# carrenD/Medical-Cross-Modality-Domain-Adaptation

Measured on NVIDIA H100. Metric: slices_per_sec_full_adversarial_step_256x256x3, higher is better.
Workload: dtype f32 (wgmma bf16 hi/lo split x3, fp32 accumulate)

## Files before the change

medical-cross-modality-domain-adaptation_b200/csrc/conv_tc.cu:

```cuda
#include <cuda.h>
#include <cstdio>
#include <cstdlib>
#include <cuda_bf16.h>
#include "common.cuh"
#include "../../include/pnp_b200.h"

namespace {

constexpr int BLOCK_M = 128;
constexpr int BLOCK_K = 64;
constexpr int WGMMA_K = 16;
constexpr int CONSUMER_THREADS = 256;
constexpr int CONSUMER_WARPS = CONSUMER_THREADS / 32;
constexpr int TC_THREADS = CONSUMER_THREADS + 32;

__device__ __forceinline__ uint32_t smem_u32(const void* p) { return (uint32_t)__cvta_generic_to_shared(p); }

__device__ __forceinline__ void mbar_init(uint32_t bar, uint32_t count) {
  asm volatile("mbarrier.init.shared::cta.b64 [%0], %1;" ::"r"(bar), "r"(count));
}
__device__ __forceinline__ void mbar_expect_tx(uint32_t bar, uint32_t bytes) {
  asm volatile("mbarrier.arrive.expect_tx.shared::cta.b64 _, [%0], %1;" ::"r"(bar), "r"(bytes) : "memory");
}
__device__ __forceinline__ void mbar_arrive(uint32_t bar) {
  asm volatile("mbarrier.arrive.shared::cta.b64 _, [%0];" ::"r"(bar) : "memory");
}
__device__ __forceinline__ bool mbar_try_wait(uint32_t bar, uint32_t parity) {
  uint32_t ok;
  asm volatile(
      "{\n\t.reg .pred p;\n\t"
      "mbarrier.try_wait.parity.shared::cta.b64 p, [%1], %2;\n\t"
      "selp.u32 %0, 1, 0, p;\n\t}"
      : "=r"(ok)
      : "r"(bar), "r"(parity)
      : "memory");
  return ok != 0;
}
__device__ __forceinline__ unsigned long long globaltimer_ns() {
  unsigned long long t;
  asm volatile("mov.u64 %0, %globaltimer;" : "=l"(t));
  return t;
}
__device__ __forceinline__ void mbar_wait(uint32_t bar, uint32_t parity) {
  if (mbar_try_wait(bar, parity)) return;
  unsigned long long t0 = globaltimer_ns();
  while (!mbar_try_wait(bar, parity)) {
    if (globaltimer_ns() - t0 > 4000000000ull) __trap();
  }
}
__device__ __forceinline__ void fence_barrier_init() { asm volatile("fence.mbarrier_init.release.cluster;" ::: "memory"); }
__device__ __forceinline__ void consumer_sync() { asm volatile("bar.sync 1, %0;" ::"n"(CONSUMER_THREADS) : "memory"); }

__device__ __forceinline__ void tma_load_4d(uint32_t dst, const CUtensorMap* map, uint32_t bar, int c0, int c1, int c2, int c3) {
  asm volatile(
      "cp.async.bulk.tensor.4d.shared::cluster.global.tile.mbarrier::complete_tx::bytes [%0], [%1, {%3, %4, %5, %6}], [%2];"
      ::"r"(dst), "l"(map), "r"(bar), "r"(c0), "r"(c1), "r"(c2), "r"(c3)
      : "memory");
}
__device__ __forceinline__ void tma_load_2d(uint32_t dst, const CUtensorMap* map, uint32_t bar, int c0, int c1) {
  asm volatile(
      "cp.async.bulk.tensor.2d.shared::cluster.global.tile.mbarrier::complete_tx::bytes [%0], [%1, {%3, %4}], [%2];"
      ::"r"(dst), "l"(map), "r"(bar), "r"(c0), "r"(c1)
      : "memory");
}
__device__ __forceinline__ void tma_prefetch_desc(const CUtensorMap* map) {
  asm volatile("prefetch.tensormap [%0];" ::"l"(map) : "memory");
}

__device__ __forceinline__ void wgmma_fence() { asm volatile("wgmma.fence.sync.aligned;" ::: "memory"); }
__device__ __forceinline__ void wgmma_commit() { asm volatile("wgmma.commit_group.sync.aligned;" ::: "memory"); }
template <int N>
__device__ __forceinline__ void wgmma_wait() { asm volatile("wgmma.wait_group.sync.aligned %0;" ::"n"(N) : "memory"); }
template <int R>
__device__ __forceinline__ void fence_acc(float (&d)[R]) {
#pragma unroll
  for (int i = 0; i < R; ++i) asm volatile("" : "+f"(d[i])::"memory");
}


template <int TA, int TB>
__device__ __forceinline__ void wgmma_m64n16k16(float (&d)[8], uint64_t da, uint64_t db, int scale_d) {
  asm volatile(
      "{\n\t.reg .pred p;\n\tsetp.ne.b32 p, %10, 0;\n\t"
      "wgmma.mma_async.sync.aligned.m64n16k16.f32.bf16.bf16 {"
      "%0, %1, %2, %3, %4, %5, %6, %7"
      "}, %8, %9, p, 1, 1, %11, %12;\n\t}"
      : "+f"(d[0]), "+f"(d[1]), "+f"(d[2]), "+f"(d[3]), "+f"(d[4]), "+f"(d[5]), "+f"(d[6]), "+f"(d[7])
      : "l"(da), "l"(db), "r"(scale_d), "n"(TA), "n"(TB)
      : "memory");
}
template <int TA, int TB>
__device__ __forceinline__ void wgmma_m64n32k16(float (&d)[16], uint64_t da, uint64_t db, int scale_d) {
  asm volatile(
      "{\n\t.reg .pred p;\n\tsetp.ne.b32 p, %18, 0;\n\t"
      "wgmma.mma_async.sync.aligned.m64n32k16.f32.bf16.bf16 {"
      "%0, %1, %2, %3, %4, %5, %6, %7, %8, %9, %10, %11, %12, %13, %14, %15"
      "}, %16, %17, p, 1, 1, %19, %20;\n\t}"
      : "+f"(d[0]), "+f"(d[1]), "+f"(d[2]), "+f"(d[3]), "+f"(d[4]), "+f"(d[5]), "+f"(d[6]), "+f"(d[7]),
        "+f"(d[8]), "+f"(d[9]), "+f"(d[10]), "+f"(d[11]), "+f"(d[12]), "+f"(d[13]), "+f"(d[14]), "+f"(d[15])
      : "l"(da), "l"(db), "r"(scale_d), "n"(TA), "n"(TB)
      : "memory");
}
template <int TA, int TB>
__device__ __forceinline__ void wgmma_m64n64k16(float (&d)[32], uint64_t da, uint64_t db, int scale_d) {
  asm volatile(
      "{\n\t.reg .pred p;\n\tsetp.ne.b32 p, %34, 0;\n\t"
      "wgmma.mma_async.sync.aligned.m64n64k16.f32.bf16.bf16 {"
      "%0, %1, %2, %3, %4, %5, %6, %7, %8, %9, %10, %11, %12, %13, %14, %15, "
      "%16, %17, %18, %19, %20, %21, %22, %23, %24, %25, %26, %27, %28, %29, %30, %31"
      "}, %32, %33, p, 1, 1, %35, %36;\n\t}"
      : "+f"(d[0]), "+f"(d[1]), "+f"(d[2]), "+f"(d[3]), "+f"(d[4]), "+f"(d[5]), "+f"(d[6]), "+f"(d[7]),
        "+f"(d[8]), "+f"(d[9]), "+f"(d[10]), "+f"(d[11]), "+f"(d[12]), "+f"(d[13]), "+f"(d[14]), "+f"(d[15]),
        "+f"(d[16]), "+f"(d[17]), "+f"(d[18]), "+f"(d[19]), "+f"(d[20]), "+f"(d[21]), "+f"(d[22]), "+f"(d[23]),
        "+f"(d[24]), "+f"(d[25]), "+f"(d[26]), "+f"(d[27]), "+f"(d[28]), "+f"(d[29]), "+f"(d[30]), "+f"(d[31])
      : "l"(da), "l"(db), "r"(scale_d), "n"(TA), "n"(TB)
      : "memory");
}
template <int TA, int TB>
__device__ __forceinline__ void wgmma_m64n128k16(float (&d)[64], uint64_t da, uint64_t db, int scale_d) {
  asm volatile(
      "{\n\t.reg .pred p;\n\tsetp.ne.b32 p, %66, 0;\n\t"
      "wgmma.mma_async.sync.aligned.m64n128k16.f32.bf16.bf16 {"
      "%0, %1, %2, %3, %4, %5, %6, %7, %8, %9, %10, %11, %12, %13, %14, %15, "
      "%16, %17, %18, %19, %20, %21, %22, %23, %24, %25, %26, %27, %28, %29, %30, %31, "
      "%32, %33, %34, %35, %36, %37, %38, %39, %40, %41, %42, %43, %44, %45, %46, %47, "
      "%48, %49, %50, %51, %52, %53, %54, %55, %56, %57, %58, %59, %60, %61, %62, %63"
      "}, %64, %65, p, 1, 1, %67, %68;\n\t}"
      : "+f"(d[0]), "+f"(d[1]), "+f"(d[2]), "+f"(d[3]), "+f"(d[4]), "+f"(d[5]), "+f"(d[6]), "+f"(d[7]),
        "+f"(d[8]), "+f"(d[9]), "+f"(d[10]), "+f"(d[11]), "+f"(d[12]), "+f"(d[13]), "+f"(d[14]), "+f"(d[15]),
        "+f"(d[16]), "+f"(d[17]), "+f"(d[18]), "+f"(d[19]), "+f"(d[20]), "+f"(d[21]), "+f"(d[22]), "+f"(d[23]),
        "+f"(d[24]), "+f"(d[25]), "+f"(d[26]), "+f"(d[27]), "+f"(d[28]), "+f"(d[29]), "+f"(d[30]), "+f"(d[31]),
        "+f"(d[32]), "+f"(d[33]), "+f"(d[34]), "+f"(d[35]), "+f"(d[36]), "+f"(d[37]), "+f"(d[38]), "+f"(d[39]),
        "+f"(d[40]), "+f"(d[41]), "+f"(d[42]), "+f"(d[43]), "+f"(d[44]), "+f"(d[45]), "+f"(d[46]), "+f"(d[47]),
        "+f"(d[48]), "+f"(d[49]), "+f"(d[50]), "+f"(d[51]), "+f"(d[52]), "+f"(d[53]), "+f"(d[54]), "+f"(d[55]),
// ... 40 lines not shown
  int kchunks;
  int ntaps;
  short tap_oy[MAX_TAPS], tap_ox[MAX_TAPS];
  int tap_wrow[MAX_TAPS];
  int tw, th, tn;
  int tiles_x, tiles_y, tiles_n;
  int accumulate;
  PnpDropout drop;
  double* bn_sum;
  double* bn_sumsq;
  const float* ep_scale;
  const float* ep_shift;
  const float* ep_skip;
  int ep_skip_c, ep_skip_off, ep_act;
  uint16_t* out_hi;
  uint16_t* out_lo;
  int total_tiles;
  int rot_mul;
  int taps_inner;
  int ksplit;
  int nphases;
  struct Phase {
    short tap_begin, tap_count, py, px;
    int U, V, tiles_x, tiles_y, tile_base;
  } ph[16];
};

struct TileCoord {
  int x0, y0, img0, n0, tap_begin, tap_count, U, V, py, px, kb_begin, kb_count, mt;
};

template <int BLOCK_N>
__device__ __forceinline__ TileCoord decode_tile(const TcArgs& a, int t, int n_tiles) {
  TileCoord c;
  int tiles_x = a.tiles_x, tiles_y = a.tiles_y;
  int ks = 0;
  if (a.ksplit > 1) { ks = t % a.ksplit; t /= a.ksplit; }
  c.tap_begin = 0; c.tap_count = a.ntaps; c.U = a.U; c.V = a.V; c.py = a.out_py; c.px = a.out_px;
  if (a.nphases > 0) {
    int p = 0;
    while (p + 1 < a.nphases && t >= a.ph[p + 1].tile_base) ++p;
    t -= a.ph[p].tile_base;
    tiles_x = a.ph[p].tiles_x; tiles_y = a.ph[p].tiles_y;
    c.tap_begin = a.ph[p].tap_begin; c.tap_count = a.ph[p].tap_count;
    c.U = a.ph[p].U; c.V = a.ph[p].V; c.py = a.ph[p].py; c.px = a.ph[p].px;
  }
  int mt = t / n_tiles;
  c.mt = mt;
  c.n0 = (t - mt * n_tiles) * BLOCK_N;
  const int txi = mt % tiles_x;
  mt /= tiles_x;
  const int tyi = mt % tiles_y;
  const int tni = mt / tiles_y;
  c.x0 = txi * a.tw; c.y0 = tyi * a.th; c.img0 = tni * a.tn;
  const int nkb = c.tap_count * a.kchunks;
  if (a.ksplit > 1) {
    c.kb_begin = (int)((long long)nkb * ks / a.ksplit);
    c.kb_count = (int)((long long)nkb * (ks + 1) / a.ksplit) - c.kb_begin;
  } else {
    c.kb_begin = 0; c.kb_count = nkb;
  }
  return c;
}

__device__ __forceinline__ void kblock_of(const TcArgs& a, const TileCoord& tc, int i, int kchunks, int& tap, int& kc) {
  const int rot = (tc.kb_count >= 16) ? (int)(((long long)tc.mt * a.rot_mul) % tc.kb_count) : 0;
  int kr = i + rot;
  if (kr >= tc.kb_count) kr -= tc.kb_count;
  const int kb = tc.kb_begin + kr;
  int tl;
  if (a.taps_inner) { kc = kb / tc.tap_count; tl = kb - kc * tc.tap_count; }
  else { tl = kb / kchunks; kc = kb - tl * kchunks; }
  tap = tc.tap_begin + tl;
}

template <int BLOCK_N, int NTERMS, int BK>
struct TcCfg {
  static constexpr int A_TILE_BYTES = BLOCK_M * BK * 2;
  static constexpr int B_TILE_BYTES = BLOCK_N * BK * 2;
  static constexpr int NPLANES = (NTERMS == 1) ? 1 : 2;
  static constexpr int STAGE_BYTES = NPLANES * (A_TILE_BYTES + B_TILE_BYTES);
  static constexpr int STAGES_RAW = (200 * 1024) / STAGE_BYTES;
  static constexpr int STAGES = STAGES_RAW > 8 ? 8 : STAGES_RAW;
  static constexpr int STAT_BYTES = 2 * BLOCK_N * 8;
  static constexpr int SMEM_BYTES = STAGES * STAGE_BYTES + STAT_BYTES + 1024  + 256 ;
  static_assert(STAGES >= 2, "pipeline needs two stages");
  static_assert(SMEM_BYTES <= 227 * 1024, "H100 allows 227 KB of shared memory per block");
};

__device__ __forceinline__ uint32_t word_of(const uint4& r, int k) { return k == 0 ? r.x : k == 1 ? r.y : k == 2 ? r.z : r.w; }

template <int BLOCK_N, int NTERMS, int BK>
__global__ void __launch_bounds__(TC_THREADS, 1)
conv_tc_kernel(const __grid_constant__ CUtensorMap map_a_hi, const __grid_constant__ CUtensorMap map_a_lo,
               const __grid_constant__ CUtensorMap map_b_hi, const __grid_constant__ CUtensorMap map_b_lo,
               float* __restrict__ out, TcArgs a) {
  pnp_pdl_trigger();
  using Cfg = TcCfg<BLOCK_N, NTERMS, BK>;
  constexpr int A_TILE_BYTES = Cfg::A_TILE_BYTES;
  constexpr int STAGES = Cfg::STAGES;
  constexpr int ACC = BLOCK_N / 2;
  extern __shared__ uint8_t smem_raw[];
  uint8_t* smem = reinterpret_cast<uint8_t*>((reinterpret_cast<uintptr_t>(smem_raw) + 1023) & ~(uintptr_t)1023);
  double* stat = reinterpret_cast<double*>(smem + STAGES * Cfg::STAGE_BYTES);
  uint64_t* bars = reinterpret_cast<uint64_t*>(stat + 2 * BLOCK_N);

  const int warp = threadIdx.x >> 5;
  const int lane = threadIdx.x & 31;
  const int n_tiles = a.Cout / BLOCK_N;
  const int kchunks = a.kchunks;
  const bool bn_on = a.bn_sum != nullptr;

  if (threadIdx.x == 0) {
    tma_prefetch_desc(&map_a_hi);
    tma_prefetch_desc(&map_b_hi);
    if (NTERMS > 1) { tma_prefetch_desc(&map_a_lo); tma_prefetch_desc(&map_b_lo); }
    for (int s = 0; s < STAGES; ++s) {
      mbar_init(smem_u32(&bars[s]), 1);
      mbar_init(smem_u32(&bars[STAGES + s]), CONSUMER_WARPS);
    }
    fence_barrier_init();
  }
  for (int i = threadIdx.x; i < 2 * BLOCK_N; i += TC_THREADS) stat[i] = 0.0;
  __syncthreads();
  pnp_pdl_wait();

  if (warp == CONSUMER_WARPS) {
    if (lane == 0) {
      const uint32_t box_a_bytes = (uint32_t)(a.tw * a.th * a.tn) * BK * 2;
      const uint32_t tx_bytes = Cfg::NPLANES * (box_a_bytes + (uint32_t)Cfg::B_TILE_BYTES);
      int stage = 0;
      uint32_t phase = 0;
      for (int t = blockIdx.x; t < a.total_tiles; t += gridDim.x) {
        const TileCoord tc = decode_tile<BLOCK_N>(a, t, n_tiles);
        for (int i = 0; i < tc.kb_count; ++i) {
          int tap, kc;
          kblock_of(a, tc, i, kchunks, tap, kc);
          mbar_wait(smem_u32(&bars[STAGES + stage]), phase ^ 1);
          const uint32_t full = smem_u32(&bars[stage]);
          mbar_expect_tx(full, tx_bytes);
          uint8_t* st = smem + stage * Cfg::STAGE_BYTES;
          const int cx = tc.x0 * a.in_mul + a.tap_ox[tap];
          const int cy = tc.y0 * a.in_mul + a.tap_oy[tap];
          const int wrow = a.tap_wrow[tap] + tc.n0;
          tma_load_4d(smem_u32(st), &map_a_hi, full, kc * BK, cx, cy, tc.img0);
          tma_load_2d(smem_u32(st + Cfg::NPLANES * A_TILE_BYTES), &map_b_hi, full, kc * BK, wrow);
          if (NTERMS > 1) {
            tma_load_4d(smem_u32(st + A_TILE_BYTES), &map_a_lo, full, kc * BK, cx, cy, tc.img0);
            tma_load_2d(smem_u32(st + 2 * A_TILE_BYTES + Cfg::B_TILE_BYTES), &map_b_lo, full, kc * BK, wrow);
          }
          if (++stage == STAGES) { stage = 0; phase ^= 1; }
        }
      }
    }
    return;
  }

  const int wg = warp >> 2;
  const int q = lane & 3;
  const int cq = q * 2;
  const int per_img = a.th * a.tw;
  const bool drop_on = a.drop.seed_ptr != nullptr;
  unsigned long long seed = 0ull;
  if (drop_on) seed = *a.drop.seed_ptr;
  int stat_n0 = -1;
  auto flush_stats = [&]() {
    consumer_sync();
    for (int i = threadIdx.x; i < BLOCK_N; i += CONSUMER_THREADS) {
      atomicAdd(a.bn_sum + stat_n0 + i, stat[i]);
      atomicAdd(a.bn_sumsq + stat_n0 + i, stat[BLOCK_N + i]);
      stat[i] = 0.0;
      stat[BLOCK_N + i] = 0.0;
    }
    consumer_sync();
  };

  float acc[ACC];
  int stage = 0;
  uint32_t phase = 0;
  for (int t = blockIdx.x; t < a.total_tiles; t += gridDim.x) {
    const TileCoord tc = decode_tile<BLOCK_N>(a, t, n_tiles);
    const int n0 = tc.n0;
    if (bn_on && n0 != stat_n0) {
      if (stat_n0 >= 0) flush_stats();
      stat_n0 = n0;
    }
    if (tc.kb_count == 0) {
#pragma unroll
      for (int i = 0; i < ACC; ++i) acc[i] = 0.f;
    }
    int prev = -1;
    for (int kb = 0; kb < tc.kb_count; ++kb) {
      mbar_wait(smem_u32(&bars[stage]), phase);
      wgmma_fence();
      const uint32_t st = smem_u32(smem + stage * Cfg::STAGE_BYTES);
      const uint32_t a_hi = st + wg * 64 * BK * 2;
      const uint32_t a_lo = a_hi + A_TILE_BYTES;
      const uint32_t b_hi = st + Cfg::NPLANES * A_TILE_BYTES;
      const uint32_t b_lo = b_hi + Cfg::B_TILE_BYTES;
#pragma unroll
      for (int k = 0; k < BK / WGMMA_K; ++k) {
        const uint32_t koff = k * WGMMA_K * 2;
        const uint64_t da_hi = make_kmajor_desc<BK>(a_hi + koff);
        const uint64_t db_hi = make_kmajor_desc<BK>(b_hi + koff);
        if (NTERMS > 1) {
          const uint64_t da_lo = make_kmajor_desc<BK>(a_lo + koff);
          const uint64_t db_lo = make_kmajor_desc<BK>(b_lo + koff);
          wgmma_bf16<BLOCK_N, 0, 0>(acc, da_lo, db_hi, (kb | k) != 0);
          wgmma_bf16<BLOCK_N, 0, 0>(acc, da_hi, db_lo, 1);
          wgmma_bf16<BLOCK_N, 0, 0>(acc, da_hi, db_hi, 1);
        } else {
          wgmma_bf16<BLOCK_N, 0, 0>(acc, da_hi, db_hi, (kb | k) != 0);
        }
      }
      wgmma_commit();
      wgmma_wait<1>();
      if (prev >= 0) {
        __syncwarp();
        if (lane == 0) mbar_arrive(smem_u32(&bars[STAGES + prev]));
      }
      prev = stage;
      if (++stage == STAGES) { stage = 0; phase ^= 1; }
    }
    wgmma_wait<0>();
    fence_acc(acc);
    if (prev >= 0) {
      __syncwarp();
      if (lane == 0) mbar_arrive(smem_u32(&bars[STAGES + prev]));
    }

    long long pix[2];
    bool valid[2];
#pragma unroll
    for (int h = 0; h < 2; ++h) {
      const int m = wg * 64 + (warp & 3) * 16 + (lane >> 2) + 8 * h;
      const int rni = m / per_img;
      const int rem = m - rni * per_img;
      const int ryy = rem / a.tw;
      const int img = tc.img0 + rni, u = tc.y0 + ryy, v_ = tc.x0 + (rem - ryy * a.tw);
      valid[h] = (rni < a.tn) && (img < a.B) && (u < tc.U) && (v_ < tc.V);
      const int oy = u * a.out_mul + tc.py, ox = v_ * a.out_mul + tc.px;
      pix[h] = ((long long)img * a.OH + oy) * a.OW + ox;
    }
    if (drop_on) {
#pragma unroll
      for (int h = 0; h < 2; ++h) {
        const unsigned long long blk0 = (unsigned long long)(pix[h] * a.Cout + n0 + q * 8) >> 3;
#pragma unroll
        for (int jg = 0; jg < (BLOCK_N / 8 + 3) / 4; ++jg) {
          const uint4 blk = pnp_dropout_bits8(a.drop, seed, blk0 + 4 * jg);
          uint32_t got[4];
          got[0] = word_of(blk, q);
#pragma unroll
          for (int s = 1; s < 4; ++s) got[s] = __shfl_xor_sync(0xffffffffu, word_of(blk, q ^ s), s);
#pragma unroll
          for (int jq = 0; jq < 4; ++jq) {
            const int j = 4 * jg + jq;
            if (j >= BLOCK_N / 8) break;
            const int sj = q ^ jq;
            const uint32_t w = sj == 0 ? got[0] : sj == 1 ? got[1] : sj == 2 ? got[2] : got[3];
            acc[4 * j + 2 * h] *= pnp_drop_sel(a.drop, w & 0xffffu);
            acc[4 * j + 2 * h + 1] *= pnp_drop_sel(a.drop, w >> 16);
          }
        }
      }
    }
#pragma unroll
    for (int j = 0; j < BLOCK_N / 8; ++j) {
      const int c0 = j * 8 + cq;
      const int ch = n0 + c0;
      float v[2][2];
#pragma unroll
      for (int h = 0; h < 2; ++h) {
        v[h][0] = acc[4 * j + 2 * h];
        v[h][1] = acc[4 * j + 2 * h + 1];
      }
      if (bn_on) {
        float s0 = (valid[0] ? v[0][0] : 0.f) + (valid[1] ? v[1][0] : 0.f);
        float s1 = (valid[0] ? v[0][1] : 0.f) + (valid[1] ? v[1][1] : 0.f);
        float q0 = (valid[0] ? v[0][0] * v[0][0] : 0.f) + (valid[1] ? v[1][0] * v[1][0] : 0.f);
        float q1 = (valid[0] ? v[0][1] * v[0][1] : 0.f) + (valid[1] ? v[1][1] * v[1][1] : 0.f);
#pragma unroll
        for (int off = 4; off < 32; off <<= 1) {
          s0 += __shfl_xor_sync(0xffffffffu, s0, off);
          s1 += __shfl_xor_sync(0xffffffffu, s1, off);
          q0 += __shfl_xor_sync(0xffffffffu, q0, off);
          q1 += __shfl_xor_sync(0xffffffffu, q1, off);
        }
        if (lane < 4) {
          atomicAdd(stat + c0, (double)s0);
          atomicAdd(stat + c0 + 1, (double)s1);
          atomicAdd(stat + BLOCK_N + c0, (double)q0);
          atomicAdd(stat + BLOCK_N + c0 + 1, (double)q1);
        }
      }
      float2 sc = make_float2(1.f, 1.f), sh = make_float2(0.f, 0.f);
      if (a.ep_scale != nullptr) {
        sc = __ldg(reinterpret_cast<const float2*>(a.ep_scale + ch));
        sh = __ldg(reinterpret_cast<const float2*>(a.ep_shift + ch));
      }
      const bool skip_on = a.ep_skip != nullptr && ch >= a.ep_skip_off && ch < a.ep_skip_off + a.ep_skip_c;
#pragma unroll
      for (int h = 0; h < 2; ++h) {
        if (!valid[h]) continue;
        float2 o = make_float2(v[h][0], v[h][1]);
        if (a.ep_scale != nullptr) { o.x = fmaf(o.x, sc.x, sh.x); o.y = fmaf(o.y, sc.y, sh.y); }
        if (skip_on) {
          const float2 sk = __ldg(reinterpret_cast<const float2*>(a.ep_skip + pix[h] * a.ep_skip_c - a.ep_skip_off + ch));
          o.x += sk.x; o.y += sk.y;
        }
        constexpr float kMinNormal = 1.17549435e-38f;
        if (a.ep_act == PNP_ACT_RELU) {
          o.x = o.x >= kMinNormal ? o.x : 0.f; o.y = o.y >= kMinNormal ? o.y : 0.f;
        } else if (a.ep_act == PNP_ACT_LRELU) {
          o.x = o.x >= kMinNormal ? o.x : (o.x > 0.f ? 0.f : 0.2f * o.x);
          o.y = o.y >= kMinNormal ? o.y : (o.y > 0.f ? 0.f : 0.2f * o.y);
        }
        const long long e0 = pix[h] * a.Cout + ch;
        if (out != nullptr) {
          float2* dst = reinterpret_cast<float2*>(out + e0);
          if (a.ksplit > 1) {
            atomicAdd(dst, o);
          } else {
            if (a.accumulate) {
              const float2 p = *dst;
              o.x += p.x; o.y += p.y;
            }
            *dst = o;
          }
        }
        if (a.out_hi != nullptr) {
          uint16_t h0, l0, h1, l1;
          split1(o.x, h0, l0);
          split1(o.y, h1, l1);
          *reinterpret_cast<uint32_t*>(a.out_hi + e0) = (uint32_t)h0 | ((uint32_t)h1 << 16);
          if (a.out_lo) *reinterpret_cast<uint32_t*>(a.out_lo + e0) = (uint32_t)l0 | ((uint32_t)l1 << 16);
        }
      }
    }
  }
  if (bn_on && stat_n0 >= 0) flush_stats();
}



__global__ void __launch_bounds__(256)
split_bf16_kernel(const float* __restrict__ x, uint16_t* __restrict__ hi, uint16_t* __restrict__ lo, long long n) {
  pnp_pdl_enter();
  long long n4 = n >> 2;
  for (long long i = (long long)blockIdx.x * 256 + threadIdx.x; i < n4; i += (long long)gridDim.x * 256) {
    float4 v = __ldg(reinterpret_cast<const float4*>(x) + i);
    ushort4 h, l;
    split1(v.x, h.x, l.x); split1(v.y, h.y, l.y); split1(v.z, h.z, l.z); split1(v.w, h.w, l.w);
    reinterpret_cast<ushort4*>(hi)[i] = h;
    if (lo) reinterpret_cast<ushort4*>(lo)[i] = l;
  }
  if (blockIdx.x == 0 && threadIdx.x < (n & 3)) {
    long long i = (n4 << 2) + threadIdx.x;
    uint16_t h, l;
    split1(x[i], h, l);
    hi[i] = h;
    if (lo) lo[i] = l;
  }
}

__global__ void __launch_bounds__(256)
split_bf16_pad_kernel(const float* __restrict__ x, uint16_t* __restrict__ hi, uint16_t* __restrict__ lo, long long rows, int C,
                      int Cpad) {
  pnp_pdl_enter();
  const int q4 = Cpad >> 2;
  long long total = rows * q4;
  for (long long i = (long long)blockIdx.x * 256 + threadIdx.x; i < total; i += (long long)gridDim.x * 256) {
    long long r = i / q4;
    int c = (int)(i - r * q4) * 4;
    ushort4 h = make_ushort4(0, 0, 0, 0), l = make_ushort4(0, 0, 0, 0);
    if (c < C) {
      float4 v = __ldg(reinterpret_cast<const float4*>(x + r * C + c));
      split1(v.x, h.x, l.x); split1(v.y, h.y, l.y); split1(v.z, h.z, l.z); split1(v.w, h.w, l.w);
    }
    reinterpret_cast<ushort4*>(hi)[i] = h;
    if (lo) reinterpret_cast<ushort4*>(lo)[i] = l;
  }
}

__global__ void __launch_bounds__(256)
split_weight_kernel(const float* __restrict__ w, uint16_t* __restrict__ hi, uint16_t* __restrict__ lo, int taps, int Cin,
                    int Cout, int for_dgrad, int CinP) {
  pnp_pdl_enter();
  __shared__ float tile[32][33];
  const int tap = blockIdx.z;
  const float* src = w + (long long)tap * Cin * Cout;
  if (for_dgrad) {
    long long obase = (long long)tap * Cin * Cout;
    int ci = blockIdx.y * 32 + threadIdx.y * 4;
    int co = blockIdx.x * 32 + threadIdx.x;
    for (int r = 0; r < 4; ++r) {
      if (ci + r < Cin && co < Cout) {
        uint16_t h, l;
        split1(src[(long long)(ci + r) * Cout + co], h, l);
        hi[obase + (long long)(ci + r) * Cout + co] = h;
        if (lo) lo[obase + (long long)(ci + r) * Cout + co] = l;
// ... 177 lines not shown
    wgmma_commit();
    wgmma_wait<1>();
    if (prev >= 0) {
      __syncwarp();
      if (lane == 0) mbar_arrive(smem_u32(&bars[STAGES + prev]));
    }
    prev = stage;
    if (++stage == STAGES) { stage = 0; phase ^= 1; }
  }
  wgmma_wait<0>();
  fence_acc(acc);

  const int cq = (lane & 3) * 2;
#pragma unroll
  for (int h = 0; h < 2; ++h) {
    const int m = wg * 64 + (warp & 3) * 16 + (lane >> 2) + 8 * h;
    int ci = ci0 + m, tap_w = tap;
    if (a.pack == 2) { tap_w = tap * 2 + (m >> 6); ci = m & 63; }
    else if (a.pack == 4) { tap_w = tap * 4 + (m >> 5); ci = m & 31; }
    if (ci >= a.Cin || tap_w >= a.ntaps) continue;
    float* orow = a.dw + ((long long)tap_w * a.Cin + ci) * a.Cout + co0 + cq;
#pragma unroll
    for (int j = 0; j < BLOCK_N / 8; ++j)
      atomicAdd(reinterpret_cast<float2*>(orow + j * 8), make_float2(acc[4 * j + 2 * h], acc[4 * j + 2 * h + 1]));
  }
}

int make_act_map(CUtensorMap* m, const uint16_t* ptr, int B, int H, int W, int C, int tw, int th, int tn, int stride, int bk = BLOCK_K) {
  EncodeTiledFn fn = get_encode_fn();
  if (!fn) return PNP_ERR_DRIVER;
  if (tw * stride > 256 || th * stride > 256 || tn > 256) return PNP_ERR_UNSUPPORTED;
  cuuint64_t dims[4] = {(cuuint64_t)C, (cuuint64_t)W, (cuuint64_t)H, (cuuint64_t)B};
  cuuint64_t strides[3] = {(cuuint64_t)C * 2, (cuuint64_t)W * C * 2, (cuuint64_t)H * W * C * 2};
  cuuint32_t box[4] = {(cuuint32_t)bk, (cuuint32_t)(tw * stride), (cuuint32_t)(th * stride), (cuuint32_t)tn};
  cuuint32_t estr[4] = {1, (cuuint32_t)stride, (cuuint32_t)stride, 1};
  CUresult r = fn(m, CU_TENSOR_MAP_DATA_TYPE_BFLOAT16, 4, (void*)ptr, dims, strides, box, estr, CU_TENSOR_MAP_INTERLEAVE_NONE,
                  bk == 64 ? CU_TENSOR_MAP_SWIZZLE_128B : (bk == 32 ? CU_TENSOR_MAP_SWIZZLE_64B : CU_TENSOR_MAP_SWIZZLE_32B), CU_TENSOR_MAP_L2_PROMOTION_L2_128B, CU_TENSOR_MAP_FLOAT_OOB_FILL_NONE);
  return r == CUDA_SUCCESS ? PNP_OK : PNP_ERR_DRIVER;
}

int make_w_map(CUtensorMap* m, const uint16_t* ptr, long long rows, int K, int block_n, int bk = BLOCK_K) {
  EncodeTiledFn fn = get_encode_fn();
  if (!fn) return PNP_ERR_DRIVER;
  cuuint64_t dims[2] = {(cuuint64_t)K, (cuuint64_t)rows};
  cuuint64_t strides[1] = {(cuuint64_t)K * 2};
  cuuint32_t box[2] = {(cuuint32_t)bk, (cuuint32_t)block_n};
  cuuint32_t estr[2] = {1, 1};
  CUresult r = fn(m, CU_TENSOR_MAP_DATA_TYPE_BFLOAT16, 2, (void*)ptr, dims, strides, box, estr, CU_TENSOR_MAP_INTERLEAVE_NONE,
                  bk == 64 ? CU_TENSOR_MAP_SWIZZLE_128B : (bk == 32 ? CU_TENSOR_MAP_SWIZZLE_64B : CU_TENSOR_MAP_SWIZZLE_32B), CU_TENSOR_MAP_L2_PROMOTION_L2_256B, CU_TENSOR_MAP_FLOAT_OOB_FILL_NONE);
  return r == CUDA_SUCCESS ? PNP_OK : PNP_ERR_DRIVER;
}

int choose_tile(int U, int V, int B, int rows, int exact, int* tw, int* th, int* tn) {
  if (V >= rows) {
    if (V % rows != 0) return PNP_ERR_UNSUPPORTED;
    *tw = rows; *th = 1; *tn = 1;
    return PNP_OK;
  }
  *tw = V;
  *th = rows / V;
  if (*th > U) *th = U;
  *tn = (*th == U) ? (rows / (*tw * *th)) : 1;
  if (*tn < 1) *tn = 1;
  if (exact) {
    if ((*tw) * (*th) * (*tn) != rows || (U % *th) != 0) return PNP_ERR_UNSUPPORTED;
  } else if (*tn > B) {
    *tn = B;
  }
  return PNP_OK;
}

int g_last_cfg[3] = {0, 0, 0};

int sm_count() {
  static int num_sms = 0;
  if (num_sms == 0) {
    int dev = 0;
    if (cudaGetDevice(&dev) != cudaSuccess || cudaDeviceGetAttribute(&num_sms, cudaDevAttrMultiProcessorCount, dev) != cudaSuccess)
      num_sms = PNP_NUM_SMS;
  }
  return num_sms;
}

template <int BLOCK_N, int NTERMS, int BK>
int launch_tc(const CUtensorMap& ma_hi, const CUtensorMap& ma_lo, const CUtensorMap& mb_hi, const CUtensorMap& mb_lo,
              float* y, const TcArgs& a, cudaStream_t s) {
  using Cfg = TcCfg<BLOCK_N, NTERMS, BK>;
  static bool attr_set = false;
  if (!attr_set) {
    PNP_CUDA(cudaFuncSetAttribute(conv_tc_kernel<BLOCK_N, NTERMS, BK>, cudaFuncAttributeMaxDynamicSharedMemorySize, Cfg::SMEM_BYTES));
    attr_set = true;
  }
  const int num_sms = sm_count();
  const long long tiles = a.total_tiles;
  dim3 grid((unsigned)(tiles < num_sms ? tiles : num_sms));
  pnp_launch(conv_tc_kernel<BLOCK_N, NTERMS, BK>, grid, TC_THREADS, Cfg::SMEM_BYTES, s, ma_hi, ma_lo, mb_hi, mb_lo, y, a);
  PNP_LAUNCH_CHECK();
  return PNP_OK;
}

template <int BLOCK_N, int NTERMS>
int launch_wg(const CUtensorMap& mx_hi, const CUtensorMap& mx_lo, const CUtensorMap& md_hi, const CUtensorMap& md_lo,
              const WgArgs& a, int splits, cudaStream_t s) {
  using Cfg = WgCfg<BLOCK_N, NTERMS>;
  static bool attr_set = false;
  if (!attr_set) {
    PNP_CUDA(cudaFuncSetAttribute(conv_wgrad_tc_kernel<BLOCK_N, NTERMS>, cudaFuncAttributeMaxDynamicSharedMemorySize, Cfg::SMEM_BYTES));
    attr_set = true;
  }
  dim3 grid(a.ngroups * a.mt * a.nt, splits);
  pnp_launch(conv_wgrad_tc_kernel<BLOCK_N, NTERMS>, grid, TC_THREADS, Cfg::SMEM_BYTES, s, mx_hi, mx_lo, md_hi, md_lo, a);
  PNP_LAUNCH_CHECK();
  return PNP_OK;
}

PnpDropout make_drop(const pnp_dropout_cfg* d) { return pnp_make_drop(d); }

int run_tc(const uint16_t* a_hi, const uint16_t* a_lo, int AH, int AW, int a_stride, const uint16_t* w_hi, const uint16_t* w_lo,
           long long w_rows, float* out, TcArgs& a, int nterms, cudaStream_t s) {
  int rc = choose_tile(a.U, a.V, a.B, BLOCK_M, 0, &a.tw, &a.th, &a.tn);
  if (rc) return rc;
  a.tiles_x = pnp_cdiv(a.V, a.tw);
  if (a.nphases == 0 && a.V % a.tw != 0) return PNP_ERR_UNSUPPORTED;
  a.tiles_y = pnp_cdiv(a.U, a.th);
  a.tiles_n = pnp_cdiv(a.B, a.tn);
  const int block_n = (a.Cout % 128 == 0) ? 128 : ((a.Cout % 64 == 0) ? 64 : ((a.Cout % 32 == 0) ? 32 : 16));
  int bk = (a.Cin % 64 == 0) ? 64 : ((a.Cin % 32 == 0) ? 32 : 16);
  {
    static int bk128_env = -1, bk64_env = -1;
    if (bk128_env < 0) { const char* e = getenv("PNP_TC_BK128"); bk128_env = e ? atoi(e) : 64; }
    if (bk64_env < 0) { const char* e = getenv("PNP_TC_BK64"); bk64_env = e ? atoi(e) : 64; }
    if (block_n == 128 && bk == 64 && bk128_env == 32) bk = 32;
    if (block_n == 64 && bk == 64 && bk64_env == 32) bk = 32;
  }
  a.kchunks = a.Cin / bk;
  g_last_cfg[0] = block_n; g_last_cfg[1] = bk; g_last_cfg[2] = 1;
  {
    const int n_tiles = a.Cout / block_n;
    if (a.nphases == 0) {
      a.total_tiles = a.tiles_x * a.tiles_y * a.tiles_n * n_tiles;
    } else {
      int base = 0;
      for (int p = 0; p < a.nphases; ++p) {
        a.ph[p].tiles_x = pnp_cdiv(a.ph[p].V, a.tw);
        a.ph[p].tiles_y = pnp_cdiv(a.ph[p].U, a.th);
        a.ph[p].tile_base = base;
        base += a.ph[p].tiles_x * a.ph[p].tiles_y * a.tiles_n * n_tiles;
      }
      a.total_tiles = base;
    }
  }
  {
    static int rot_env = -1;
    static int order_env = -1;
    if (rot_env < 0) { const char* e = getenv("PNP_TC_ROT"); rot_env = e ? atoi(e) : 7; }
    if (order_env < 0) { const char* e = getenv("PNP_TC_ORDER"); order_env = e ? atoi(e) : 0; }
    a.rot_mul = rot_env;
    a.taps_inner = order_env;
  }
  a.ksplit = 1;
  double* bn_sum_after = nullptr;
  double* bn_sumsq_after = nullptr;
  {
    int min_taps = a.ntaps;
    for (int p = 0; p < a.nphases; ++p) min_taps = a.ph[p].tap_count < min_taps ? a.ph[p].tap_count : min_taps;
    const int min_kb = min_taps * a.kchunks;
    const int sms = sm_count();
    const bool fused_ep = a.ep_scale != nullptr || a.ep_skip != nullptr || a.ep_act != PNP_ACT_NONE || a.out_hi != nullptr;
    if (!fused_ep && a.total_tiles * 2 <= sms && min_kb >= 8) {
      int ks = sms / a.total_tiles;
      if (ks > min_kb / 4) ks = min_kb / 4;
      if (ks > 32) ks = 32;
      if (ks > 1) {
        a.ksplit = ks;
        g_last_cfg[2] = ks;
        a.total_tiles *= ks;
        if (!a.accumulate) PNP_CUDA(cudaMemsetAsync(out, 0, sizeof(float) * (size_t)a.B * a.OH * a.OW * a.Cout, s));
        bn_sum_after = a.bn_sum; bn_sumsq_after = a.bn_sumsq;
        a.bn_sum = nullptr; a.bn_sumsq = nullptr;
      }
    }
  }
  CUtensorMap ma_hi, ma_lo, mb_hi, mb_lo;
  rc = make_act_map(&ma_hi, a_hi, a.B, AH, AW, a.Cin, a.tw, a.th, a.tn, a_stride, bk);
  if (rc) return rc;
  rc = make_w_map(&mb_hi, w_hi, w_rows, a.Cin, block_n, bk);
  if (rc) return rc;
  if (nterms == 3) {
    rc = make_act_map(&ma_lo, a_lo, a.B, AH, AW, a.Cin, a.tw, a.th, a.tn, a_stride, bk);
    if (rc) return rc;
    rc = make_w_map(&mb_lo, w_lo, w_rows, a.Cin, block_n, bk);
    if (rc) return rc;
  } else {
    ma_lo = ma_hi;
    mb_lo = mb_hi;
  }
#define PNP_TC_GO(N_, K_)                                                                                  \
  rc = (nterms == 3) ? launch_tc<N_, 3, K_>(ma_hi, ma_lo, mb_hi, mb_lo, out, a, s)                         \
                     : launch_tc<N_, 1, K_>(ma_hi, ma_lo, mb_hi, mb_lo, out, a, s)
  if (block_n == 128 && bk == 64) { PNP_TC_GO(128, 64); }
  else if (block_n == 128 && bk == 32) { PNP_TC_GO(128, 32); }
  else if (block_n == 64 && bk == 64) { PNP_TC_GO(64, 64); }
  else if (block_n == 64 && bk == 32) { PNP_TC_GO(64, 32); }
  else if (block_n == 32 && bk == 64) { PNP_TC_GO(32, 64); }
  else if (block_n == 32 && bk == 32) { PNP_TC_GO(32, 32); }
  else if (block_n == 32 && bk == 16) { PNP_TC_GO(32, 16); }
  else if (block_n == 16 && bk == 16) { PNP_TC_GO(16, 16); }
  else if (block_n == 16 && bk == 32) { PNP_TC_GO(16, 32); }
  else return PNP_ERR_UNSUPPORTED;
#undef PNP_TC_GO
  if (rc) return rc;
  if (bn_sum_after) return pnp_bn_stats(out, (long long)a.B * a.OH * a.OW, a.Cout, bn_sum_after, bn_sumsq_after, (void*)s);
  return PNP_OK;
}

bool tc_geom_ok(const pnp_conv_geom* g) {
  return g && g->B > 0 && g->H > 0 && g->W > 0 && g->Ho > 0 && g->Wo > 0 && g->kh > 0 && g->kw > 0 && g->dil > 0 && g->stride > 0 &&
         g->kh * g->kw <= MAX_TAPS && (g->Cin % 64 == 0 || g->Cin == 32 || g->Cin == 16) &&
         (g->Cout % 64 == 0 || g->Cout == 32 || g->Cout == 16);
}

}

extern "C" int pnp_tc_last_config(int* block_n, int* block_k, int* ksplit) {
  if (block_n) *block_n = g_last_cfg[0];
  if (block_k) *block_k = g_last_cfg[1];
  if (ksplit) *ksplit = g_last_cfg[2];
  return PNP_OK;
}

extern "C" int pnp_tc_available(void) {
  int dev = 0;
  if (cudaGetDevice(&dev) != cudaSuccess) return 0;
  int major = 0;
  if (cudaDeviceGetAttribute(&major, cudaDevAttrComputeCapabilityMajor, dev) != cudaSuccess) return 0;
  return (major == 9 && get_encode_fn() != nullptr) ? 1 : 0;
}

extern "C" int pnp_split_bf16(const float* x, uint16_t* hi, uint16_t* lo, long long n, void* stream) {
  if (!x || !hi || n <= 0) return PNP_ERR_BAD_ARG;
  long long blocks = (n / 4 + 255) / 256;
  if (blocks < 1) blocks = 1;
  if (blocks > PNP_NUM_SMS * 32LL) blocks = PNP_NUM_SMS * 32LL;
  pnp_launch(split_bf16_kernel, (unsigned)blocks, 256, 0, (cudaStream_t)stream, x, hi, lo, n);
  PNP_LAUNCH_CHECK();
  return PNP_OK;
}

extern "C" int pnp_split_bf16_pad(const float* x, uint16_t* hi, uint16_t* lo, long long rows, int C, int Cpad, void* stream) {
  if (!x || !hi || rows <= 0 || C <= 0 || Cpad < C || (C % 4) != 0 || (Cpad % 4) != 0) return PNP_ERR_BAD_ARG;
  long long blocks = (rows * (Cpad / 4) + 255) / 256;
  if (blocks > PNP_NUM_SMS * 32LL) blocks = PNP_NUM_SMS * 32LL;
  pnp_launch(split_bf16_pad_kernel, (unsigned)blocks, 256, 0, (cudaStream_t)stream, x, hi, lo, rows, C, Cpad);
  PNP_LAUNCH_CHECK();
  return PNP_OK;
}

extern "C" int pnp_split_weight_bf16(const float* w, uint16_t* hi, uint16_t* lo, int kh, int kw, int Cin, int Cout,
                                     int for_dgrad, int cin_pad, void* stream) {
  if (!w || !hi || kh <= 0 || kw <= 0 || Cin <= 0 || Cout <= 0) return PNP_ERR_BAD_ARG;
  const int CinP = (cin_pad > Cin) ? cin_pad : Cin;
  if (for_dgrad && CinP != Cin) return PNP_ERR_UNSUPPORTED;
  dim3 grid(pnp_cdiv(Cout, 32), pnp_cdiv(CinP, 32), kh * kw);
  pnp_launch(split_weight_kernel, grid, dim3(32, 8), 0, (cudaStream_t)stream, w, hi, lo, kh * kw, Cin, Cout, for_dgrad, CinP);
  PNP_LAUNCH_CHECK();
  return PNP_OK;
}

extern "C" int pnp_conv2d_tc_fwd_fused(const uint16_t* x_hi, const uint16_t* x_lo, const uint16_t* w_hi, const uint16_t* w_lo,
                                       float* y, const pnp_conv_geom* g, int nterms, const pnp_dropout_cfg* drop, int accumulate,
                                       double* bn_sum, double* bn_sumsq, const pnp_tc_epilogue* ep, void* stream) {
  if (!g || !x_hi || !w_hi) return PNP_ERR_BAD_ARG;
  if (!y && !(ep && ep->y_hi)) return PNP_ERR_BAD_ARG;
  if (nterms != 1 && nterms != 3) return PNP_ERR_BAD_ARG;
  if (nterms == 3 && (!x_lo || !w_lo)) return PNP_ERR_BAD_ARG;
  if ((bn_sum == nullptr) != (bn_sumsq == nullptr)) return PNP_ERR_BAD_ARG;
  if (accumulate && bn_sum) return PNP_ERR_BAD_ARG;
  if (!tc_geom_ok(g)) return PNP_ERR_UNSUPPORTED;
  TcArgs a;
  a.B = g->B; a.OH = g->Ho; a.OW = g->Wo; a.Cout = g->Cout; a.Cin = g->Cin;
  a.U = g->Ho; a.V = g->Wo; a.out_mul = 1; a.out_py = 0; a.out_px = 0; a.in_mul = g->stride; a.nphases = 0;
  a.ntaps = g->kh * g->kw;
// ... 155 lines not shown
```

Before: 471.6.

## Add ping-pong warpgroup schedule to conv tensor-core kernel for narrow tiles

Adds a ping-pong variant of the persistent conv kernel for BLOCK_N<=64 with more tiles than SMs. Each of two consumer warpgroups computes a whole 128-row tile and they alternate tiles, handing off mainloop turns through named barriers so one warpgroup's epilogue overlaps the other's wgmma. The producer warpgroup gives up registers via setmaxnreg and the consumers take more, and BN stat scratch is split per warpgroup. The cost is doubled accumulator registers per thread, extra barrier traffic, and trickier stage/phase bookkeeping, since each warpgroup has to skip the other's k-blocks.

Result: faster. 484.2, median of 6 (+2.7%).

```diff
diff --git a/medical-cross-modality-domain-adaptation_b200/csrc/conv_tc.cu b/medical-cross-modality-domain-adaptation_b200/csrc/conv_tc.cu
--- a/medical-cross-modality-domain-adaptation_b200/csrc/conv_tc.cu
+++ b/medical-cross-modality-domain-adaptation_b200/csrc/conv_tc.cu
@@ -13,6 +13,7 @@
 constexpr int CONSUMER_THREADS = 256;
 constexpr int CONSUMER_WARPS = CONSUMER_THREADS / 32;
 constexpr int TC_THREADS = CONSUMER_THREADS + 32;
+constexpr int PP_THREADS = CONSUMER_THREADS + 128;
 
 __device__ __forceinline__ uint32_t smem_u32(const void* p) { return (uint32_t)__cvta_generic_to_shared(p); }
 
@@ -49,7 +50,13 @@
   }
 }
 __device__ __forceinline__ void fence_barrier_init() { asm volatile("fence.mbarrier_init.release.cluster;" ::: "memory"); }
-__device__ __forceinline__ void consumer_sync() { asm volatile("bar.sync 1, %0;" ::"n"(CONSUMER_THREADS) : "memory"); }
+__device__ __forceinline__ void wg_sync(int wg) { asm volatile("bar.sync %0, 128;" ::"r"(1 + wg) : "memory"); }
+__device__ __forceinline__ void turn_wait(int wg) { asm volatile("bar.sync %0, 256;" ::"r"(3 + wg) : "memory"); }
+__device__ __forceinline__ void turn_pass(int wg) { asm volatile("bar.arrive %0, 256;" ::"r"(3 + (wg ^ 1)) : "memory"); }
+template <int N>
+__device__ __forceinline__ void setmaxnreg_dec() { asm volatile("setmaxnreg.dec.sync.aligned.u32 %0;" ::"n"(N)); }
+template <int N>
+__device__ __forceinline__ void setmaxnreg_inc() { asm volatile("setmaxnreg.inc.sync.aligned.u32 %0;" ::"n"(N)); }
 
 __device__ __forceinline__ void tma_load_4d(uint32_t dst, const CUtensorMap* map, uint32_t bar, int c0, int c1, int c2, int c3) {
   asm volatile(
@@ -256,7 +263,7 @@
   static constexpr int STAGE_BYTES = NPLANES * (A_TILE_BYTES + B_TILE_BYTES);
   static constexpr int STAGES_RAW = (200 * 1024) / STAGE_BYTES;
   static constexpr int STAGES = STAGES_RAW > 8 ? 8 : STAGES_RAW;
-  static constexpr int STAT_BYTES = 2 * BLOCK_N * 8;
+  static constexpr int STAT_BYTES = 2 * 2 * BLOCK_N * 8;
   static constexpr int SMEM_BYTES = STAGES * STAGE_BYTES + STAT_BYTES + 1024  + 256 ;
   static_assert(STAGES >= 2, "pipeline needs two stages");
   static_assert(SMEM_BYTES <= 227 * 1024, "H100 allows 227 KB of shared memory per block");
@@ -264,8 +271,8 @@
 
 __device__ __forceinline__ uint32_t word_of(const uint4& r, int k) { return k == 0 ? r.x : k == 1 ? r.y : k == 2 ? r.z : r.w; }
 
-template <int BLOCK_N, int NTERMS, int BK>
-__global__ void __launch_bounds__(TC_THREADS, 1)
+template <int BLOCK_N, int NTERMS, int BK, bool PP>
+__global__ void __launch_bounds__(PP ? PP_THREADS : TC_THREADS, 1)
 conv_tc_kernel(const __grid_constant__ CUtensorMap map_a_hi, const __grid_constant__ CUtensorMap map_a_lo,
                const __grid_constant__ CUtensorMap map_b_hi, const __grid_constant__ CUtensorMap map_b_lo,
                float* __restrict__ out, TcArgs a) {
@@ -277,10 +284,11 @@
   extern __shared__ uint8_t smem_raw[];
   uint8_t* smem = reinterpret_cast<uint8_t*>((reinterpret_cast<uintptr_t>(smem_raw) + 1023) & ~(uintptr_t)1023);
   double* stat = reinterpret_cast<double*>(smem + STAGES * Cfg::STAGE_BYTES);
-  uint64_t* bars = reinterpret_cast<uint64_t*>(stat + 2 * BLOCK_N);
+  uint64_t* bars = reinterpret_cast<uint64_t*>(stat + 4 * BLOCK_N);
 
   const int warp = threadIdx.x >> 5;
   const int lane = threadIdx.x & 31;
+  const int wg = PP ? __shfl_sync(0xffffffffu, threadIdx.x >> 7, 0) : (int)(threadIdx.x >> 7);
   const int n_tiles = a.Cout / BLOCK_N;
   const int kchunks = a.kchunks;
   const bool bn_on = a.bn_sum != nullptr;
@@ -291,16 +299,17 @@
     if (NTERMS > 1) { tma_prefetch_desc(&map_a_lo); tma_prefetch_desc(&map_b_lo); }
     for (int s = 0; s < STAGES; ++s) {
       mbar_init(smem_u32(&bars[s]), 1);
-      mbar_init(smem_u32(&bars[STAGES + s]), CONSUMER_WARPS);
+      mbar_init(smem_u32(&bars[STAGES + s]), PP ? CONSUMER_WARPS / 2 : CONSUMER_WARPS);
     }
     fence_barrier_init();
   }
-  for (int i = threadIdx.x; i < 2 * BLOCK_N; i += TC_THREADS) stat[i] = 0.0;
+  for (int i = threadIdx.x; i < 4 * BLOCK_N; i += blockDim.x) stat[i] = 0.0;
   __syncthreads();
   pnp_pdl_wait();
 
-  if (warp == CONSUMER_WARPS) {
-    if (lane == 0) {
+  if (wg == 2) {
+    if constexpr (PP) setmaxnreg_dec<40>();
+    if (warp == CONSUMER_WARPS && lane == 0) {
       const uint32_t box_a_bytes = (uint32_t)(a.tw * a.th * a.tn) * BK * 2;
       const uint32_t tx_bytes = Cfg::NPLANES * (box_a_bytes + (uint32_t)Cfg::B_TILE_BYTES);
       int stage = 0;
@@ -330,29 +339,41 @@
     return;
   }
 
-  const int wg = warp >> 2;
+  if constexpr (PP) setmaxnreg_inc<232>();
+  constexpr int NH = PP ? 2 : 1;
+  const int h_first = PP ? 0 : wg;
   const int q = lane & 3;
   const int cq = q * 2;
   const int per_img = a.th * a.tw;
   const bool drop_on = a.drop.seed_ptr != nullptr;
   unsigned long long seed = 0ull;
   if (drop_on) seed = *a.drop.seed_ptr;
+  double* wstat = stat + wg * 2 * BLOCK_N;
   int stat_n0 = -1;
   auto flush_stats = [&]() {
-    consumer_sync();
-    for (int i = threadIdx.x; i < BLOCK_N; i += CONSUMER_THREADS) {
-      atomicAdd(a.bn_sum + stat_n0 + i, stat[i]);
-      atomicAdd(a.bn_sumsq + stat_n0 + i, stat[BLOCK_N + i]);
-      stat[i] = 0.0;
-      stat[BLOCK_N + i] = 0.0;
-    }
-    consumer_sync();
+    wg_sync(wg);
+    for (int i = threadIdx.x & 127; i < BLOCK_N; i += 128) {
+      atomicAdd(a.bn_sum + stat_n0 + i, wstat[i]);
+      atomicAdd(a.bn_sumsq + stat_n0 + i, wstat[BLOCK_N + i]);
+      wstat[i] = 0.0;
+      wstat[BLOCK_N + i] = 0.0;
+    }
+    wg_sync(wg);
   };
 
-  float acc[ACC];
+  float acc[NH][ACC];
   int stage = 0;
   uint32_t phase = 0;
-  for (int t = blockIdx.x; t < a.total_tiles; t += gridDim.x) {
+  auto skip_kblocks = [&](int t_other) {
+    if (t_other >= a.total_tiles) return;
+    stage += decode_tile<BLOCK_N>(a, t_other, n_tiles).kb_count;
+    phase ^= (uint32_t)(stage / STAGES) & 1u;
+    stage %= STAGES;
+  };
+  if (PP && wg == 1) skip_kblocks(blockIdx.x);
+  for (int pos = PP ? wg : 0;; pos += PP ? 2 : 1) {
+    const int t = blockIdx.x + pos * gridDim.x;
+    if (t >= a.total_tiles) break;
     const TileCoord tc = decode_tile<BLOCK_N>(a, t, n_tiles);
     const int n0 = tc.n0;
     if (bn_on && n0 != stat_n0) {
@@ -361,30 +382,38 @@
     }
     if (tc.kb_count == 0) {
 #pragma unroll
-      for (int i = 0; i < ACC; ++i) acc[i] = 0.f;
-    }
+      for (int i = 0; i < ACC; ++i) {
+#pragma unroll
+        for (int hh = 0; hh < NH; ++hh) acc[hh][i] = 0.f;
+      }
+    }
+    if (PP && pos > 0) turn_wait(wg);
     int prev = -1;
     for (int kb = 0; kb < tc.kb_count; ++kb) {
       mbar_wait(smem_u32(&bars[stage]), phase);
       wgmma_fence();
       const uint32_t st = smem_u32(smem + stage * Cfg::STAGE_BYTES);
-      const uint32_t a_hi = st + wg * 64 * BK * 2;
+      const uint32_t a_hi = st + h_first * 64 * BK * 2;
       const uint32_t a_lo = a_hi + A_TILE_BYTES;
       const uint32_t b_hi = st + Cfg::NPLANES * A_TILE_BYTES;
       const uint32_t b_lo = b_hi + Cfg::B_TILE_BYTES;
+      constexpr uint32_t HALF = 64 * BK * 2;
 #pragma unroll
       for (int k = 0; k < BK / WGMMA_K; ++k) {
         const uint32_t koff = k * WGMMA_K * 2;
-        const uint64_t da_hi = make_kmajor_desc<BK>(a_hi + koff);
         const uint64_t db_hi = make_kmajor_desc<BK>(b_hi + koff);
+        const int acc_d = (kb | k) != 0;
         if (NTERMS > 1) {
-          const uint64_t da_lo = make_kmajor_desc<BK>(a_lo + koff);
           const uint64_t db_lo = make_kmajor_desc<BK>(b_lo + koff);
-          wgmma_bf16<BLOCK_N, 0, 0>(acc, da_lo, db_hi, (kb | k) != 0);
-          wgmma_bf16<BLOCK_N, 0, 0>(acc, da_hi, db_lo, 1);
-          wgmma_bf16<BLOCK_N, 0, 0>(acc, da_hi, db_hi, 1);
+          wgmma_bf16<BLOCK_N, 0, 0>(acc[0], make_kmajor_desc<BK>(a_lo + koff), db_hi, acc_d);
+          if constexpr (NH > 1) wgmma_bf16<BLOCK_N, 0, 0>(acc[1], make_kmajor_desc<BK>(a_lo + HALF + koff), db_hi, acc_d);
+          wgmma_bf16<BLOCK_N, 0, 0>(acc[0], make_kmajor_desc<BK>(a_hi + koff), db_lo, 1);
+          if constexpr (NH > 1) wgmma_bf16<BLOCK_N, 0, 0>(acc[1], make_kmajor_desc<BK>(a_hi + HALF + koff), db_lo, 1);
+          wgmma_bf16<BLOCK_N, 0, 0>(acc[0], make_kmajor_desc<BK>(a_hi + koff), db_hi, 1);
+          if constexpr (NH > 1) wgmma_bf16<BLOCK_N, 0, 0>(acc[1], make_kmajor_desc<BK>(a_hi + HALF + koff), db_hi, 1);
         } else {
-          wgmma_bf16<BLOCK_N, 0, 0>(acc, da_hi, db_hi, (kb | k) != 0);
+          wgmma_bf16<BLOCK_N, 0, 0>(acc[0], make_kmajor_desc<BK>(a_hi + koff), db_hi, acc_d);
+          if constexpr (NH > 1) wgmma_bf16<BLOCK_N, 0, 0>(acc[1], make_kmajor_desc<BK>(a_hi + HALF + koff), db_hi, acc_d);
         }
       }
       wgmma_commit();
@@ -396,30 +425,34 @@
       prev = stage;
       if (++stage == STAGES) { stage = 0; phase ^= 1; }
     }
+    if (PP && t + (int)gridDim.x < a.total_tiles) turn_pass(wg);
     wgmma_wait<0>();
-    fence_acc(acc);
+#pragma unroll
+    for (int hh = 0; hh < NH; ++hh) fence_acc(acc[hh]);
     if (prev >= 0) {
       __syncwarp();
       if (lane == 0) mbar_arrive(smem_u32(&bars[STAGES + prev]));
     }
-
-    long long pix[2];
-    bool valid[2];
-#pragma unroll
-    for (int h = 0; h < 2; ++h) {
-      const int m = wg * 64 + (warp & 3) * 16 + (lane >> 2) + 8 * h;
+    if (PP) skip_kblocks(t + gridDim.x);
+
+    long long pix[2 * NH];
+    bool valid[2 * NH];
+#pragma unroll
+    for (int r = 0; r < 2 * NH; ++r) {
+      const int m = (h_first + (r >> 1)) * 64 + (warp & 3) * 16 + (lane >> 2) + 8 * (r & 1);
       const int rni = m / per_img;
       const int rem = m - rni * per_img;
       const int ryy = rem / a.tw;
       const int img = tc.img0 + rni, u = tc.y0 + ryy, v_ = tc.x0 + (rem - ryy * a.tw);
-      valid[h] = (rni < a.tn) && (img < a.B) && (u < tc.U) && (v_ < tc.V);
+      valid[r] = (rni < a.tn) && (img < a.B) && (u < tc.U) && (v_ < tc.V);
       const int oy = u * a.out_mul + tc.py, ox = v_ * a.out_mul + tc.px;
-      pix[h] = ((long long)img * a.OH + oy) * a.OW + ox;
+      pix[r] = ((long long)img * a.OH + oy) * a.OW + ox;
     }
     if (drop_on) {
 #pragma unroll
-      for (int h = 0; h < 2; ++h) {
-        const unsigned long long blk0 = (unsigned long long)(pix[h] * a.Cout + n0 + q * 8) >> 3;
+      for (int r = 0; r < 2 * NH; ++r) {
+        const int h = r & 1;
+        const unsigned long long blk0 = (unsigned long long)(pix[r] * a.Cout + n0 + q * 8) >> 3;
 #pragma unroll
         for (int jg = 0; jg < (BLOCK_N / 8 + 3) / 4; ++jg) {
           const uint4 blk = pnp_dropout_bits8(a.drop, seed, blk0 + 4 * jg);
@@ -433,8 +466,8 @@
             if (j >= BLOCK_N / 8) break;
             const int sj = q ^ jq;
             const uint32_t w = sj == 0 ? got[0] : sj == 1 ? got[1] : sj == 2 ? got[2] : got[3];
-            acc[4 * j + 2 * h] *= pnp_drop_sel(a.drop, w & 0xffffu);
-            acc[4 * j + 2 * h + 1] *= pnp_drop_sel(a.drop, w >> 16);
+            acc[r >> 1][4 * j + 2 * h] *= pnp_drop_sel(a.drop, w & 0xffffu);
+            acc[r >> 1][4 * j + 2 * h + 1] *= pnp_drop_sel(a.drop, w >> 16);
           }
         }
       }
@@ -443,17 +476,21 @@
     for (int j = 0; j < BLOCK_N / 8; ++j) {
       const int c0 = j * 8 + cq;
       const int ch = n0 + c0;
-      float v[2][2];
-#pragma unroll
-      for (int h = 0; h < 2; ++h) {
-        v[h][0] = acc[4 * j + 2 * h];
-        v[h][1] = acc[4 * j + 2 * h + 1];
+      float v[2 * NH][2];
+#pragma unroll
+      for (int r = 0; r < 2 * NH; ++r) {
+        v[r][0] = acc[r >> 1][4 * j + 2 * (r & 1)];
+        v[r][1] = acc[r >> 1][4 * j + 2 * (r & 1) + 1];
       }
       if (bn_on) {
-        float s0 = (valid[0] ? v[0][0] : 0.f) + (valid[1] ? v[1][0] : 0.f);
-        float s1 = (valid[0] ? v[0][1] : 0.f) + (valid[1] ? v[1][1] : 0.f);
-        float q0 = (valid[0] ? v[0][0] * v[0][0] : 0.f) + (valid[1] ? v[1][0] * v[1][0] : 0.f);
-        float q1 = (valid[0] ? v[0][1] * v[0][1] : 0.f) + (valid[1] ? v[1][1] * v[1][1] : 0.f);
+        float s0 = 0.f, s1 = 0.f, q0 = 0.f, q1 = 0.f;
+#pragma unroll
+        for (int r = 0; r < 2 * NH; ++r) {
+          s0 += valid[r] ? v[r][0] : 0.f;
+          s1 += valid[r] ? v[r][1] : 0.f;
+          q0 += valid[r] ? v[r][0] * v[r][0] : 0.f;
+          q1 += valid[r] ? v[r][1] * v[r][1] : 0.f;
+        }
 #pragma unroll
         for (int off = 4; off < 32; off <<= 1) {
           s0 += __shfl_xor_sync(0xffffffffu, s0, off);
@@ -462,10 +499,10 @@
           q1 += __shfl_xor_sync(0xffffffffu, q1, off);
         }
         if (lane < 4) {
-          atomicAdd(stat + c0, (double)s0);
-          atomicAdd(stat + c0 + 1, (double)s1);
-          atomicAdd(stat + BLOCK_N + c0, (double)q0);
-          atomicAdd(stat + BLOCK_N + c0 + 1, (double)q1);
+          atomicAdd(wstat + c0, (double)s0);
+          atomicAdd(wstat + c0 + 1, (double)s1);
+          atomicAdd(wstat + BLOCK_N + c0, (double)q0);
+          atomicAdd(wstat + BLOCK_N + c0 + 1, (double)q1);
         }
       }
       float2 sc = make_float2(1.f, 1.f), sh = make_float2(0.f, 0.f);
@@ -475,12 +512,12 @@
       }
       const bool skip_on = a.ep_skip != nullptr && ch >= a.ep_skip_off && ch < a.ep_skip_off + a.ep_skip_c;
 #pragma unroll
-      for (int h = 0; h < 2; ++h) {
-        if (!valid[h]) continue;
-        float2 o = make_float2(v[h][0], v[h][1]);
+      for (int r = 0; r < 2 * NH; ++r) {
+        if (!valid[r]) continue;
+        float2 o = make_float2(v[r][0], v[r][1]);
         if (a.ep_scale != nullptr) { o.x = fmaf(o.x, sc.x, sh.x); o.y = fmaf(o.y, sc.y, sh.y); }
         if (skip_on) {
-          const float2 sk = __ldg(reinterpret_cast<const float2*>(a.ep_skip + pix[h] * a.ep_skip_c - a.ep_skip_off + ch));
+          const float2 sk = __ldg(reinterpret_cast<const float2*>(a.ep_skip + pix[r] * a.ep_skip_c - a.ep_skip_off + ch));
           o.x += sk.x; o.y += sk.y;
         }
         constexpr float kMinNormal = 1.17549435e-38f;
@@ -490,7 +527,7 @@
           o.x = o.x >= kMinNormal ? o.x : (o.x > 0.f ? 0.f : 0.2f * o.x);
           o.y = o.y >= kMinNormal ? o.y : (o.y > 0.f ? 0.f : 0.2f * o.y);
         }
-        const long long e0 = pix[h] * a.Cout + ch;
+        const long long e0 = pix[r] * a.Cout + ch;
         if (out != nullptr) {
           float2* dst = reinterpret_cast<float2*>(out + e0);
           if (a.ksplit > 1) {
@@ -834,21 +871,30 @@
   return num_sms;
 }
 
-template <int BLOCK_N, int NTERMS, int BK>
+template <int BLOCK_N, int NTERMS, int BK, bool PP>
 int launch_tc(const CUtensorMap& ma_hi, const CUtensorMap& ma_lo, const CUtensorMap& mb_hi, const CUtensorMap& mb_lo,
               float* y, const TcArgs& a, cudaStream_t s) {
   using Cfg = TcCfg<BLOCK_N, NTERMS, BK>;
   static bool attr_set = false;
   if (!attr_set) {
-    PNP_CUDA(cudaFuncSetAttribute(conv_tc_kernel<BLOCK_N, NTERMS, BK>, cudaFuncAttributeMaxDynamicSharedMemorySize, Cfg::SMEM_BYTES));
+    PNP_CUDA(cudaFuncSetAttribute(conv_tc_kernel<BLOCK_N, NTERMS, BK, PP>, cudaFuncAttributeMaxDynamicSharedMemorySize, Cfg::SMEM_BYTES));
     attr_set = true;
   }
   const int num_sms = sm_count();
   const long long tiles = a.total_tiles;
   dim3 grid((unsigned)(tiles < num_sms ? tiles : num_sms));
-  pnp_launch(conv_tc_kernel<BLOCK_N, NTERMS, BK>, grid, TC_THREADS, Cfg::SMEM_BYTES, s, ma_hi, ma_lo, mb_hi, mb_lo, y, a);
+  pnp_launch(conv_tc_kernel<BLOCK_N, NTERMS, BK, PP>, grid, PP ? PP_THREADS : TC_THREADS, Cfg::SMEM_BYTES, s, ma_hi, ma_lo, mb_hi, mb_lo, y, a);
   PNP_LAUNCH_CHECK();
   return PNP_OK;
+}
+
+template <int BLOCK_N, int NTERMS, int BK>
+int launch_tc_sched(bool pp, const CUtensorMap& ma_hi, const CUtensorMap& ma_lo, const CUtensorMap& mb_hi,
+                    const CUtensorMap& mb_lo, float* y, const TcArgs& a, cudaStream_t s) {
+  if constexpr (BLOCK_N <= 64) {
+    if (pp) return launch_tc<BLOCK_N, NTERMS, BK, true>(ma_hi, ma_lo, mb_hi, mb_lo, y, a, s);
+  }
+  return launch_tc<BLOCK_N, NTERMS, BK, false>(ma_hi, ma_lo, mb_hi, mb_lo, y, a, s);
 }
 
 template <int BLOCK_N, int NTERMS>
@@ -947,9 +993,10 @@
     ma_lo = ma_hi;
     mb_lo = mb_hi;
   }
+  const bool pp = block_n <= 64 && a.total_tiles > sm_count();
 #define PNP_TC_GO(N_, K_)                                                                                  \
-  rc = (nterms == 3) ? launch_tc<N_, 3, K_>(ma_hi, ma_lo, mb_hi, mb_lo, out, a, s)                         \
-                     : launch_tc<N_, 1, K_>(ma_hi, ma_lo, mb_hi, mb_lo, out, a, s)
+  rc = (nterms == 3) ? launch_tc_sched<N_, 3, K_>(pp, ma_hi, ma_lo, mb_hi, mb_lo, out, a, s)                \
+                     : launch_tc_sched<N_, 1, K_>(pp, ma_hi, ma_lo, mb_hi, mb_lo, out, a, s)
   if (block_n == 128 && bk == 64) { PNP_TC_GO(128, 64); }
   else if (block_n == 128 && bk == 32) { PNP_TC_GO(128, 32); }
   else if (block_n == 64 && bk == 64) { PNP_TC_GO(64, 64); }
```
